# finsberg/fenicsx-beat

Measured on AMD Instinct MI355X. Metric: node_updates_per_sec, higher is better.
Workload: dtype f64

## Files before the change

### fenicsx-beat_amd/csrc/beat_ode.hip

```cpp
#include "beat_ode_kernel.h"
#include "beat_ode_jit.h"

#include <functional>


template <class Model>
static int launch_ode_run(beat_ctx* ctx, double* states, int64_t n, int64_t ld, const double* host_params,
                          int num_params, const double* ppn, int64_t pld, double t0, double dt, int64_t nsteps,
                          int nbeats, int save_freq, const int* track_idx, int ntrack, double* trace) {
  BEAT_REQUIRE(num_params == Model::NP || (host_params == nullptr && ppn == nullptr && Model::NP == 2),
               "model expects %d parameters, got %d", Model::NP, num_params);
  BEAT_REQUIRE(ntrack >= 0 && ntrack <= 8, "at most 8 tracked states");
  BEAT_REQUIRE(ntrack == 0 || (trace != nullptr && save_freq >= 1), "tracking needs a trace buffer and save_freq >= 1");
  ParamPack<Model::NP> prm;
  for (int k = 0; k < Model::NP; ++k) prm.p[k] = host_params ? host_params[k] : 1.0;
  typename Model::Derived drv = Model::derive(prm.p);
  TrackSpec tr{};
  tr.n = ntrack;
  for (int a = 0; a < ntrack; ++a) {
    BEAT_REQUIRE(track_idx[a] >= 0 && track_idx[a] < Model::NS, "tracked state %d out of range", track_idx[a]);
    tr.idx[a] = track_idx[a];
  }
  const unsigned grid = (unsigned)((n + BEAT_BLOCK - 1) / BEAT_BLOCK);
  if (ppn != nullptr) {
// ... 44 lines not shown
                                                        nsteps, nbeats, save_freq, host_track_idx, ntrack, dev_trace);
  });
  return rc == BEAT_NOT_BUILTIN ? unknown_model(model_id) : rc;
}

static unsigned ode_grid(int64_t n, int num_states) {
  unsigned grid = (unsigned)((n + BEAT_BLOCK - 1) / BEAT_BLOCK);
  static const int grid_cap_env = [] {
    const char* e = std::getenv("BEAT_ODE_GRID");
    return e ? std::atoi(e) : -1;
  }();
  static const int tile_min_states = [] {
    const char* e = std::getenv("BEAT_ODE_TILE_MIN_STATES");
    return e ? std::atoi(e) : 12;
  }();
  const int grid_cap = grid_cap_env >= 0 ? grid_cap_env : (num_states >= tile_min_states ? 0 : 24576);
  static const bool balance = [] {
    const char* e = std::getenv("BEAT_ODE_BALANCE");
    return !(e && e[0] == '0');
  }();
  if (grid_cap > 0 && grid > (unsigned)grid_cap) {
    const unsigned per_block = (grid + (unsigned)grid_cap - 1) / (unsigned)grid_cap;
    grid = (balance && per_block <= 8) ? (grid + per_block - 1) / per_block : (unsigned)grid_cap;
  }
  return grid;
}

template <class Model, bool PER_NODE, bool MARKED = false, bool SPARSE = false>
static auto launch_instance(bool have_pend, hipStream_t stream, unsigned grid, double* states, int64_t n, int64_t ld,
                            const ParamPack<Model::NP>& prm, const typename Model::Derived& drv, const double* ppn, int64_t pld, double t,
                            double dt, int v_index, double* v_copy, const PendingV& pend, const MarkedArgs& mk, const SparseRows& sp) {
  if (have_pend)
    BEAT_KERNEL((ode_step_kernel<Model, PER_NODE, true, MARKED, SPARSE>), dim3(grid), dim3(BEAT_BLOCK), 0, stream, states, n, ld, prm, drv,
                ppn, pld, t, dt, v_index, v_copy, pend, mk, sp);
  else
    BEAT_KERNEL((ode_step_kernel<Model, PER_NODE, false, MARKED, SPARSE>), dim3(grid), dim3(BEAT_BLOCK), 0, stream, states, n, ld, prm, drv,
                ppn, pld, t, dt, v_index, v_copy, pend, mk, sp);
}

template <class Model>
static int launch_ode(beat_ctx* ctx, double* states, int64_t n, int64_t ld, const double* host_params,
                      int num_params, const double* ppn, int64_t pld, double t, double dt,
                      int v_index, double* v_copy, const PendingV& pend, MarkedArgs mk = MarkedArgs{nullptr, nullptr, 0, nullptr, nullptr},
                      SparseRows sp = SparseRows{{0}, 0}) {
  BEAT_REQUIRE(num_params == Model::NP || (host_params == nullptr && ppn == nullptr && Model::NP == 2) || mk.markers != nullptr,
               "model expects %d parameters, got %d", Model::NP, num_params);
  BEAT_REQUIRE(host_params != nullptr || ppn != nullptr || mk.markers != nullptr || Model::NP == 2,
               "no parameters given: a host vector, per-node rows or parameter classes");
  if (int rc = beat_check_step_rows(Model::NS, Model::V_INDEX, v_index, v_copy, mk.markers != nullptr, pend)) return rc;
  const bool have_pend = beat_pending_has_work(pend);
  ParamPack<Model::NP> prm;
  for (int k = 0; k < Model::NP; ++k) prm.p[k] = host_params ? host_params[k] : 1.0;
  typename Model::Derived drv = Model::derive(prm.p);
  const unsigned grid = ode_grid(n, Model::NS);
  if (mk.markers != nullptr) {
    BEAT_REQUIRE(ppn == nullptr && mk.table != nullptr, "parameter classes come with a table, not with per-node rows");
    launch_instance<Model, false, true>(have_pend, ctx->stream, grid, states, n, ld, prm, drv, ppn, pld, t, dt, v_index, v_copy, pend, mk, sp);
  } else if (ppn != nullptr && sp.count > 0) {
    BEAT_REQUIRE(pld >= n, "params_ld %lld < n %lld", (long long)pld, (long long)n);
    BEAT_REQUIRE(host_params != nullptr, "sparse rows come with the uniform parameter vector");
    {
      const int rc = beat_ode_jit_launch<Model>(ctx, dim3(grid), have_pend, states, n, ld, prm, drv, ppn, pld, t, dt, v_index, v_copy, pend, mk, sp);
      if (rc != BEAT_JIT_UNAVAILABLE) return rc;
    }
    BEAT_REQUIRE(sp.count <= BEAT_MAX_SPARSE_ROWS_RT, "%d varying rows need run-time compilation, which is not available here "
                 "(beat_ode_jit_stats; at most %d rows otherwise): pass all rows (beat_ode_step)", sp.count, BEAT_MAX_SPARSE_ROWS_RT);
    launch_instance<Model, true, false, true>(have_pend, ctx->stream, grid, states, n, ld, prm, drv, ppn, pld, t, dt, v_index, v_copy, pend, mk,
                                              sp);
  } else if (ppn != nullptr) {
    BEAT_REQUIRE(pld >= n, "params_ld %lld < n %lld", (long long)pld, (long long)n);
    launch_instance<Model, true>(have_pend, ctx->stream, grid, states, n, ld, prm, drv, ppn, pld, t, dt, v_index, v_copy, pend, mk, sp);
  } else {
    launch_instance<Model, false>(have_pend, ctx->stream, grid, states, n, ld, prm, drv, ppn, pld, t, dt, v_index, v_copy, pend, mk, sp);
  }
  BEAT_LAUNCH_CHECK();
  return BEAT_OK;
}

extern "C" int beat_ode_model_info(int model_id, int* num_states, int* num_params) {
  int ns = 0, np = 0;
  const int rc = with_builtin_model(model_id, [&](auto tag) {
    using M = typename decltype(tag)::type;
    ns = M::NS;
    np = M::NP;
    return BEAT_OK;
  });
  if (rc == BEAT_NOT_BUILTIN && beat_custom_model_info(model_id, &ns, &np, nullptr) != BEAT_OK)
    return unknown_model(model_id);
  if (num_states) *num_states = ns;
  if (num_params) *num_params = np;
  return BEAT_OK;
}

static int ode_step_dispatch(beat_ctx* ctx, int model_id, double* dev_states, int64_t n, int64_t ld,
                             const double* host_params, int num_params, const double* dev_params_per_node,
                             int64_t params_ld, double t, double dt, int v_index, double* dev_v_copy,
                             const PendingV& pend, MarkedArgs mk = MarkedArgs{nullptr, nullptr, 0, nullptr, nullptr},
                             SparseRows sp = SparseRows{{0}, 0}) {
  BEAT_REQUIRE(ctx != nullptr, "null context");
  BEAT_REQUIRE(dev_states != nullptr, "null states");
  BEAT_REQUIRE(n >= 0 && ld >= n, "bad shape n=%lld ld=%lld", (long long)n, (long long)ld);
  BEAT_REQUIRE((n + BEAT_BLOCK - 1) / BEAT_BLOCK < (int64_t)0x7fffffff, "n too large");
  if (n == 0) return BEAT_OK;
  if (model_id >= BEAT_MODEL_CUSTOM_BASE) {
    BEAT_REQUIRE(sp.count == 0, "a model registered as source takes a uniform vector, all per-node rows or classes (no sparse rows)");
    int cns = 0, cnp = 0, cvi = 0;
// ... 298 lines not shown
```

### fenicsx-beat_amd/csrc/beat_ode_kernel.h

```cpp
#pragma once
#include "beat_pde_internal.h"

#include <algorithm>
#include <cmath>
#include <cstddef>
#include <cstdlib>
#include <type_traits>
#include <vector>
#include "ionic_models.h"
#include "torord_dyncl.h"


template <int NP>
struct ParamPack {
  double p[NP];
};

struct PendingV {
  const double* ring;
  int64_t fld;
  const double* alphas;
  int count;
  beat_pde_detail::GuessTerms gt;
  const double* dev_st;
// ... 39 lines not shown
};

constexpr int BEAT_MAX_SPARSE_ROWS = 16;
constexpr int BEAT_MAX_SPARSE_ROWS_RT = 4;
struct SparseRows {
  int idx[BEAT_MAX_SPARSE_ROWS];
  int count;
};

template <class Model>
struct OdeTableEntry {
  double p[Model::NP];
  typename Model::Derived d;
};

template <int... K>
struct IdxPack {
  static constexpr int count = (int)sizeof...(K);
};
template <class CT>
struct MixedParams;
template <int... K>
struct MixedParams<IdxPack<K...>> {
  const double* u;
  double v[sizeof...(K) > 0 ? sizeof...(K) : 1];
  __device__ __forceinline__ double operator[](int k) const {
    double r = u[k];
    int j = 0;
    ((r = (k == K ? v[j] : r), ++j), ...);
    return r;
  }
};
template <class D, unsigned long long DM0, unsigned long long DM1>
__device__ __forceinline__ D mix_derived(const D& du, const D& dl) {
  D d;
  constexpr int ND = (int)(sizeof(D) / sizeof(double));
  static_assert(sizeof(D) % sizeof(double) == 0 && ND <= 128, "Derived: up to 128 doubles");
  const double* a = (const double*)&du;
  const double* b = (const double*)&dl;
  double* o = (double*)&d;
#pragma unroll
  for (int j = 0; j < ND; ++j) o[j] = (((j < 64 ? DM0 : DM1) >> (j & 63)) & 1ull) ? b[j] : a[j];
  return d;
}

template <class Model, class = void>
struct beat_fm_type { using type = FastMath; };
template <class Model>
struct beat_fm_type<Model, std::void_t<typename Model::FM>> { using type = typename Model::FM; };
template <class Model, class = void>
struct beat_fm_pin_wanted : std::false_type {};
template <class Model>
struct beat_fm_pin_wanted<Model, std::void_t<decltype(Model::FM_PIN)>> : std::integral_constant<bool, Model::FM_PIN> {};
__device__ __forceinline__ double beat_any_value() {
  double x;
#ifdef __AMDGCN__
  asm volatile("" : "=v"(x));
#else
  x = 0.0;
#endif
  return x;
}
template <class Model, bool PER_NODE, bool PEND, bool MARKED = false, bool SPARSE = false, class CT = IdxPack<>,
          unsigned long long DM0 = 0, unsigned long long DM1 = 0>
__global__ __launch_bounds__(BEAT_BLOCK, (PER_NODE && CT::count == 0) ? Model::WAVES_PER_NODE : Model::WAVES) void ode_step_kernel(
    double* __restrict__ states, int64_t n, int64_t ld, ParamPack<Model::NP> prm,
    typename Model::Derived drv, const double* __restrict__ ppn, int64_t pld, double t, double dt,
    int v_index, double* __restrict__ v_copy, PendingV pend, MarkedArgs mk_arg, SparseRows sp) {
  __shared__ double etab[BEAT_EXP_TAB];
  __shared__ LogEntry ltab[128];
  static_assert(BEAT_EXP_TAB == BEAT_BLOCK, "one table entry per thread");
  etab[threadIdx.x] = beat_exp_tab_entry<beat_fm_type<Model>::type::INT_SCALE>(kExp2Tab[threadIdx.x], (int)threadIdx.x);
  if (threadIdx.x < 128) ltab[threadIdx.x] = kLogTab[threadIdx.x];
  __shared__ int cls_jn[MARKED ? BEAT_BLOCK : 1];
  __shared__ int s_pend[2];
  if (PEND && threadIdx.x == 0) {
    s_pend[0] = pend.dev_st != nullptr ? (pend.dev_st[beat_pde_detail::STOP] != 0.0 ? 1 : 0) : 1;
    s_pend[1] = pend.dev_st != nullptr ? (int)pend.dev_st[beat_pde_detail::NUPD] : -1;
  }
  __syncthreads();
  typename beat_fm_type<Model>::type fm{etab, ltab};
  if constexpr (beat_fm_pin_wanted<Model>::value) beat_fm_pin(fm);
  if (PEND && s_pend[0] == 0) return;
  const int wave_in_block = __builtin_amdgcn_readfirstlane((int)(threadIdx.x >> 6));
  for (int64_t tile = blockIdx.x;; tile += gridDim.x) {
  typedef const __attribute__((address_space(4))) char* KArgPtr;
  KArgPtr ka = (KArgPtr)__builtin_amdgcn_kernarg_segment_ptr();
  asm volatile("" : "+s"(ka));
  const PendingV& pendl = *(const PendingV*)(ka + offsetof(OdeStepKernArgHead<Model>, pend));
  const OdeStepKernArgHead<Model>& hd = *(const OdeStepKernArgHead<Model>*)ka;
  double* __restrict__ const states = hd.states;
  const int64_t n = hd.n, ld = hd.ld;
  const double* __restrict__ const ppn = hd.ppn;
  const int64_t pld = hd.pld;
  const double t = hd.t, dt = hd.dt;
  const int v_index = hd.v_index;
  double* __restrict__ const v_copy = hd.v_copy;
  (void)ppn; (void)pld; (void)v_index; (void)v_copy;
  if (tile * BEAT_BLOCK >= n) break;
  int lane_now = (int)__builtin_amdgcn_mbcnt_hi(~0u, __builtin_amdgcn_mbcnt_lo(~0u, 0u));
  asm volatile("" : "+v"(lane_now));
  const int tid = (wave_in_block << 6) + lane_now;
  const int64_t tile0 = tile * BEAT_BLOCK;
  unsigned lane_off = (unsigned)tid * 8u;
  const int64_t i = tile0 + tid;
  if (i >= n) break;
// ... 79 lines not shown
    NodeIOPending<Model::V_INDEX> io{states + tile0, ldl, lane_off, v_copy != nullptr ? v_copy + tile0 : nullptr, now.count, {}, {}, 0.0, 0.0, 0.0, 0.0, {}};
#pragma unroll
    for (int j = 0; j < BEAT_MAX_PENDING; ++j) {
      io.pp[j] = j < now.count ? __builtin_nontemporal_load(beat_at(pendl.ring + ((int64_t)j * pendl.fld + tile0), lane_off)) : beat_any_value();
      io.pa[j] = j < now.count ? pendl.alphas[j] : 0.0;
    }
    io.ge = io.gd = io.gp0 = io.gp1 = 0.0;
    if (now.gt.d != nullptr) {
      now.gt.d += tile0;
      now.gt.e += tile0;
      if (now.gt.dp[0] != nullptr) now.gt.dp[0] += tile0;
      if (now.gt.dp[1] != nullptr) now.gt.dp[1] += tile0;
      io.gt = now.gt;
      io.ge = beat_pde_detail::beat_guess_needs_e(now.gt) ? __builtin_nontemporal_load(beat_at(now.gt.e, lane_off)) : beat_any_value();
      io.gd = beat_pde_detail::beat_guess_needs_d(now.gt) ? __builtin_nontemporal_load(beat_at(now.gt.d, lane_off)) : beat_any_value();
      io.gp0 = beat_pde_detail::beat_guess_needs_dp(now.gt, 0) ? __builtin_nontemporal_load(beat_at(now.gt.dp[0], lane_off)) : beat_any_value();
      io.gp1 = beat_pde_detail::beat_guess_needs_dp(now.gt, 1) ? __builtin_nontemporal_load(beat_at(now.gt.dp[1], lane_off)) : beat_any_value();
    }
    if constexpr (PER_NODE && SPARSE && CT::count > 0) {
      MixedParams<CT> mp;
      mp.u = p_uni;
#pragma unroll
      for (int j = 0; j < CT::count; ++j) mp.v[j] = *beat_at(beat_row(ppn + tile0, j, pld), lane_off);
      if constexpr (DM0 == 0 && DM1 == 0) {
        Model::step(io, mp, d_uni, fm, t, dt);
      } else {
        const typename Model::Derived dlane = Model::derive(mp);
        const typename Model::Derived dm = mix_derived<typename Model::Derived, DM0, DM1>(d_uni, dlane);
        Model::step(io, mp, dm, fm, t, dt);
      }
    } else if (PER_NODE) {
      double pl[Model::NP];
      if (SPARSE) {
        const double* pv = p_uni;
        asm volatile("" : "+v"(pv));
#pragma unroll
        for (int k = 0; k < Model::NP; ++k) pl[k] = pv[k];
#pragma unroll
        for (int j = 0; j < BEAT_MAX_SPARSE_ROWS_RT; ++j) {
          if (j < sp.count) {
            const double vj = *beat_at(beat_row(ppn + tile0, j, pld), lane_off);
            int ij = sp.idx[j];
            asm volatile("" : "+s"(ij));
#pragma unroll
            for (int k = 0; k < Model::NP; ++k) pl[k] = k == ij ? vj : pl[k];
          }
        }
      } else {
#pragma unroll
        for (int k = 0; k < Model::NP; ++k) pl[k] = *beat_at(beat_row(ppn + tile0, k, pld), lane_off);
      }
      const typename Model::Derived dl = Model::derive(pl);
      Model::step(io, pl, dl, fm, t, dt);
    } else {
      Model::step(io, p_uni, d_uni, fm, t, dt);
    }
  } else {
    const NodeIO io{states + tile0, ldl, lane_off, nullptr, -1};
    if constexpr (PER_NODE && SPARSE && CT::count > 0) {
      MixedParams<CT> mp;
      mp.u = p_uni;
#pragma unroll
      for (int j = 0; j < CT::count; ++j) mp.v[j] = *beat_at(beat_row(ppn + tile0, j, pld), lane_off);
      if constexpr (DM0 == 0 && DM1 == 0) {
        Model::step(io, mp, d_uni, fm, t, dt);
      } else {
        const typename Model::Derived dlane = Model::derive(mp);
        const typename Model::Derived dm = mix_derived<typename Model::Derived, DM0, DM1>(d_uni, dlane);
        Model::step(io, mp, dm, fm, t, dt);
      }
    } else if (PER_NODE) {
      double pl[Model::NP];
      if (SPARSE) {
        const double* pv = p_uni;
        asm volatile("" : "+v"(pv));
#pragma unroll
        for (int k = 0; k < Model::NP; ++k) pl[k] = pv[k];
#pragma unroll
        for (int j = 0; j < BEAT_MAX_SPARSE_ROWS_RT; ++j) {
          if (j < sp.count) {
            const double vj = *beat_at(beat_row(ppn + tile0, j, pld), lane_off);
            int ij = sp.idx[j];
            asm volatile("" : "+s"(ij));
#pragma unroll
            for (int k = 0; k < Model::NP; ++k) pl[k] = k == ij ? vj : pl[k];
          }
        }
      } else {
#pragma unroll
        for (int k = 0; k < Model::NP; ++k) pl[k] = *beat_at(beat_row(ppn + tile0, k, pld), lane_off);
      }
      const typename Model::Derived dl = Model::derive(pl);
      Model::step(io, pl, dl, fm, t, dt);
    } else {
      Model::step(io, p_uni, d_uni, fm, t, dt);
    }
    if (v_copy != nullptr) v_copy[i] = states[(int64_t)v_index * ldl + i];
  }
  }
}

struct TrackSpec {
  int idx[8];
  int n;
};

template <class Model, bool PER_NODE>
__global__ __launch_bounds__(BEAT_BLOCK, 1) void ode_run_kernel(
    double* __restrict__ states, int64_t n, int64_t ld, ParamPack<Model::NP> prm, typename Model::Derived drv,
    const double* __restrict__ ppn, int64_t pld, double t0, double dt, int64_t nsteps, int nbeats, int save_freq,
    TrackSpec track, double* __restrict__ trace) {
  __shared__ double etab[BEAT_EXP_TAB];
  __shared__ LogEntry ltab[128];
  static_assert(BEAT_EXP_TAB == BEAT_BLOCK, "one table entry per thread");
  etab[threadIdx.x] = beat_exp_tab_entry<beat_fm_type<Model>::type::INT_SCALE>(kExp2Tab[threadIdx.x], (int)threadIdx.x);
  if (threadIdx.x < 128) ltab[threadIdx.x] = kLogTab[threadIdx.x];
  __syncthreads();
  typename beat_fm_type<Model>::type fm{etab, ltab};
  if constexpr (beat_fm_pin_wanted<Model>::value) beat_fm_pin(fm);
  const int64_t i = (int64_t)blockIdx.x * BEAT_BLOCK + threadIdx.x;
  if (i >= n) return;
  double y[Model::NS];
#pragma unroll
  for (int k = 0; k < Model::NS; ++k) y[k] = states[(int64_t)k * ld + i];
  double pl[PER_NODE ? Model::NP : 1];
  typename Model::Derived dl = drv;
  if (PER_NODE) {
#pragma unroll
    for (int k = 0; k < Model::NP; ++k) pl[k] = ppn[(int64_t)k * pld + i];
    dl = Model::derive((const double*)pl);
  }
  const RegIO rio{y};
  const NodeIO gio{states + (int64_t)blockIdx.x * BEAT_BLOCK, ld, threadIdx.x * 8u, nullptr, -1};
  int64_t row = 0;
  for (int beat = 0; beat < nbeats; ++beat) {
    for (int64_t j = 0; j < nsteps; ++j) {
      if (track.n > 0 && j % save_freq == 0) {
        for (int a = 0; a < track.n; ++a) {
          double v = 0.0;
#pragma unroll
          for (int k = 0; k < Model::NS; ++k)
            if (k == track.idx[a]) v = y[k];
          trace[(row * track.n + a) * n + i] = v;
        }
        ++row;
      }
// ... 23 lines not shown
```

### fenicsx-beat_amd/csrc/ionic_models.h

```cpp
#pragma once

#include <cmath>
#include <type_traits>
#include <utility>

#include "beat_common.h"


constexpr int BEAT_EXP_TAB = 256;
__device__ const double kExp2Tab[BEAT_EXP_TAB] = {
    1.0, 1.0027112750502025, 1.0054299011128027, 1.0081558981184175,
    1.0108892860517005, 1.0136300849514894, 1.016378314910953, 1.019133996077738,
    1.0218971486541166, 1.0246677928971357, 1.0274459491187637, 1.030231637686041,
    1.0330248790212284, 1.0358256936019572, 1.0386341019613787, 1.041450124688316,
    1.0442737824274138, 1.0471050958792898, 1.0499440858006872, 1.0527907730046264,
    1.0556451783605572, 1.0585073227945128, 1.061377227289262, 1.0642549128844645,
    1.0671404006768237, 1.0700337118202419, 1.0729348675259756, 1.075843889062791,
    1.0787607977571199, 1.0816856149932152, 1.0846183622133092, 1.0875590609177697,
    1.0905077326652577, 1.0934643990728858, 1.0964290818163769, 1.099401802630222,
    1.102382583307841, 1.1053714457017412, 1.1083684117236787, 1.1113735033448175,
    1.1143867425958924, 1.1174081515673693, 1.1204377524096067, 1.12347556733302,
    1.1265216186082418, 1.129575928566288, 1.1326385195987192, 1.1357094141578055,
    1.1387886347566916, 1.1418762039695616, 1.1449721444318042, 1.148076478840179,
    1.1511892299529827, 1.154310420590216, 1.1574400736337511, 1.1605782120274988,
// ... 194 lines not shown
template <bool INT_SCALE>
__device__ __forceinline__ double beat_clamp_exp_arg(double x) {
  return fmin(fmax(x, BEAT_EXP_LO), INT_SCALE ? BEAT_EXP_HI_INT : BEAT_EXP_HI);
}
__device__ __forceinline__ double beat_exp_overflow(double x, double e) { return x > BEAT_EXP_HI ? HUGE_VAL : e; }
template <bool INT_SCALE>
__device__ __forceinline__ double beat_exp_tab_entry(double t, int j) {
#ifdef __AMDGCN__
  if constexpr (INT_SCALE) return __hiloint2double(__double2hiint(t) - (j << 12), __double2loint(t));
#endif
  (void)j;
  return t;
}

__device__ __forceinline__ double beat_rcp(double x) {
  const double r = __builtin_amdgcn_rcp(x);
  const double e = fma(-x, r, 1.0);
  return fma(r, fma(e, e, e), r);
}

__device__ __forceinline__ double beat_rsqrt(double x) {
  const double r = __builtin_amdgcn_rsq(x);
  const double e = fma(-(x * r), r, 1.0);
  return fma(r * fma(e, 0.375, 0.5), e, r);
}

__device__ __forceinline__ double beat_frexp_mant(double x) {
#ifdef __AMDGCN__
  return __builtin_amdgcn_frexp_mant(x);
#else
  int e;
  return std::frexp(x, &e);
#endif
}
__device__ __forceinline__ int beat_frexp_exp(double x) {
#ifdef __AMDGCN__
  return __builtin_amdgcn_frexp_exp(x);
#else
  int e = 0;
  return std::isfinite(x) ? (std::frexp(x, &e), e) : 0;
#endif
}
__device__ __forceinline__ bool beat_pos_finite(double x) {
#ifdef __AMDGCN__
  return __builtin_amdgcn_class(x, 0x180);
#else
  return x > 0.0 && x < HUGE_VAL;
#endif
}
__device__ __forceinline__ double beat_log_special(double x) {
  const double y = x + 0.0;
  return y - __builtin_amdgcn_rsq(y);
}

__device__ __forceinline__ double beat_sconst(double c) {
#ifdef __AMDGCN__
  asm volatile("" : "+s"(c));
#endif
  return c;
}

template <bool INT_SCALE_>
struct FastMathT {
  static constexpr bool INT_SCALE = INT_SCALE_;
  const double* __restrict__ tab;
  const LogEntry* __restrict__ ltab;
  double magic = 6755399441055744.0;
  __device__ __forceinline__ double log(double x) const {
    const double xm = beat_frexp_mant(x);
    const int hi = __double2hiint(xm);
    const int e = beat_frexp_exp(x) - 1;
    const LogEntry t = ltab[(hi >> 13) & 127];
    const double m = __hiloint2double((hi & 0x000fffff) | 0x3ff00000, __double2loint(xm));
    const double r = fma(m, t.inv, -1.0);
    double p = fma(r, -1.0 / 6.0, 1.0 / 5.0);
    p = fma(r, p, -0.25);
    p = fma(r, p, 1.0 / 3.0);
    p = fma(r, p, -0.5);
    p = fma(r * r, p, r);
    const double ed = (double)e;
    const double es = __hiloint2double(beat_pos_finite(x) ? __double2hiint(ed) : __double2hiint(beat_log_special(x)), __double2loint(ed));
    return fma(es, 0.693147180559663, t.logc + fma(es, 2.8235290563031577e-13, p));
  }
  __device__ __forceinline__ double exp(double x) const {
    const double kb = fma(x, 369.3299304675746, magic);
    const double k = kb - magic;
    double r = fma(k, -0.002707606173999011, x);
    r = fma(k, -6.327543041662719e-14, r);
    const int ki = __double2loint(kb);
    const double t = tab[ki & (BEAT_EXP_TAB - 1)];
    const double r2 = r * r;
    double p = fma(r, beat_sconst(1.0 / 6.0), 0.5);
    p = fma(r2, beat_sconst(1.0 / 24.0), p);
    p = fma(r2, p, r);
#ifdef __AMDGCN__
    if constexpr (INT_SCALE) {
      const double ts = __hiloint2double(__double2hiint(t) + (int)((unsigned)ki << 12), __double2loint(t));
      return fma(ts, p, ts);
    }
#endif
    return ldexp(fma(t, p, t), ki >> 8);
  }
};

using FastMath = FastMathT<false>;
template <bool I>
__device__ __forceinline__ void beat_fm_pin(FastMathT<I>& fm) {
#ifdef __AMDGCN__
  asm volatile("" : "+v"(fm.magic));
#endif
}

__device__ __forceinline__ double beat_guard(double v) { return fabs(v) < 1.0e-4 ? copysign(1.0e-4, v) : v; }

__device__ __forceinline__ double beat_row_load(const double* p) {
#ifdef __clang__
  return __builtin_nontemporal_load(p);
#else
  return *p;
#endif
}
__device__ __forceinline__ void beat_row_store(double* p, double v) {
#ifdef __clang__
  __builtin_nontemporal_store(v, p);
#else
  *p = v;
#endif
}

template <class T>
__device__ __forceinline__ T* beat_row(T* base, int k, int64_t ld) {
#ifdef __AMDGCN__
  asm volatile("" : "+s"(ld));
#endif
  return base + (int64_t)k * ld;
// ... 4 lines not shown
#ifdef __AMDGCN__
  asm volatile("" : "+v"(byte_off));
#endif
  return (T*)((Byte*)uniform_base + byte_off);
}
struct NodeIO {
  double* __restrict__ base;
  int64_t ld;
  mutable unsigned i;
  double* __restrict__ v_copy;
  int v_index;
  __device__ __forceinline__ double load(int k) const { return beat_row_load(beat_at(beat_row(base, k, ld), i)); }
  __device__ __forceinline__ void store(int k, double v) const {
    beat_row_store(beat_at(beat_row(base, k, ld), i), v);
    if (v_copy != nullptr && k == v_index) *beat_at(v_copy, i) = v;
  }
};

constexpr int BEAT_MAX_PENDING = 6;
constexpr int BEAT_MAX_PENDING_CLASS = 12;
template <int VIDX>
struct NodeIOPending {
  double* __restrict__ base;
  int64_t ld;
  mutable unsigned i;
  double* __restrict__ v_copy;
  int npend;
  double pa[BEAT_MAX_PENDING], pp[BEAT_MAX_PENDING];
  double ge, gd, gp0, gp1;
  beat_pde_detail::GuessTerms gt;
  __device__ __forceinline__ double load(int k) const {
    double x = beat_row_load(beat_at(beat_row(base, k, ld), i));
    if (k == VIDX) {
      if (gt.d != nullptr) {
        double inc = (!gt.accumulate && gt.use_e) ? ge : 0.0;
#pragma unroll
        for (int j = 0; j < BEAT_MAX_PENDING; ++j)
          if (j < npend) inc = fma(pa[j], pp[j], inc);
        beat_pde_detail::beat_guess_record(gt, beat_at(gt.d, i), beat_at(gt.e, i), inc, gd, gp0, gp1, ge);
        return x + inc;
      }
#pragma unroll
      for (int j = 0; j < BEAT_MAX_PENDING; ++j)
        if (j < npend) x = fma(pa[j], pp[j], x);
    }
    return x;
  }
  __device__ __forceinline__ void store(int k, double v) const {
    beat_row_store(beat_at(beat_row(base, k, ld), i), v);
    if (k == VIDX && v_copy != nullptr) *beat_at(v_copy, i) = v;
  }
};

struct RegIO {
  double* y;
  __device__ __forceinline__ double load(int k) const { return y[k]; }
  __device__ __forceinline__ void store(int k, double v) const { y[k] = v; }
};

struct SimpleOde {
  static constexpr int NS = 2, NP = 2, V_INDEX = 0;
  static constexpr bool REGISTER_LOOP = true;
  static constexpr int WAVES = BEAT_ODE_WAVES;
  static constexpr int WAVES_PER_NODE = BEAT_ODE_WAVES_PER_NODE;
  struct Derived {};
  __host__ __device__ static Derived derive(const double*) { return {}; }
  template <class IO>
  __device__ static __forceinline__ void step(const IO& io, const double* p, const Derived&, const FastMath&,
                                              double, double dt) {
    const double v = io.load(0), s = io.load(1);
    io.store(0, v - p[0] * s * dt);
    io.store(1, s + p[1] * v * dt);
  }
};

struct FhnDemo {
  static constexpr int NS = 2, NP = 10, V_INDEX = 1;
  static constexpr bool REGISTER_LOOP = true;
  static constexpr int WAVES = BEAT_ODE_WAVES;
  static constexpr int WAVES_PER_NODE = BEAT_ODE_WAVES_PER_NODE;
  struct Derived {};
  __host__ __device__ static Derived derive(const double*) { return {}; }
  template <class IO>
  __device__ static __forceinline__ void step(const IO& io, const double* p, const Derived&, const FastMath&,
                                              double t, double dt) {
    const double s = io.load(0), V = io.load(1);
    const double V_peak = p[0], V_rest = p[1], a = p[2], b = p[3], c_1 = p[4], c_2 = p[5],
                 c_3 = p[6], stim_amplitude = p[7], stim_duration = p[8], stim_start = p[9];
    const double V_amp = V_peak - V_rest;
    const double i_Stim = (t >= stim_start && t <= stim_start + stim_duration) ? stim_amplitude : 0.0;
    const double ds_dt = b * (-c_3 * s + (V - V_rest));
    const double V_th = V_amp * a + V_rest;
    const double I = -s * (c_2 / V_amp) * (V - V_rest) +
                     (((c_1 / (V_amp * V_amp)) * (V - V_rest)) * (V - V_th)) * (-V + V_peak);
    const double dV_dt = I + i_Stim;
    io.store(0, s + dt * ds_dt);
    io.store(1, V + dt * dV_dt);
  }
};

struct FhnReadme {
  static constexpr int NS = 2, NP = 11, V_INDEX = 1;
  static constexpr bool REGISTER_LOOP = true;
  static constexpr int WAVES = BEAT_ODE_WAVES;
  static constexpr int WAVES_PER_NODE = BEAT_ODE_WAVES_PER_NODE;
  struct Derived {};
  __host__ __device__ static Derived derive(const double*) { return {}; }
  template <class IO>
  __device__ static __forceinline__ void step(const IO& io, const double* p, const Derived&, const FastMath&,
                                              double t, double dt) {
    const double s = io.load(0), v = io.load(1);
    const double c_1 = p[0], c_2 = p[1], c_3 = p[2], a = p[3], b = p[4], v_amp = p[5],
                 v_rest = p[6], v_peak = p[7], stim_amplitude = p[8], stim_duration = p[9],
                 stim_start = p[10];
    const double i_app = (t > stim_start && t < stim_start + stim_duration) ? stim_amplitude : 0.0;
    const double ds_dt = b * (-c_3 * s + (v - v_rest));
    const double v_th = v_amp * a + v_rest;
    const double I = -s * (c_2 / v_amp) * (v - v_rest) +
                     (((c_1 / (v_amp * v_amp)) * (v - v_rest)) * (v - v_th)) * (-v + v_peak);
    const double dV_dt = I + i_app;
    io.store(0, ds_dt * dt + s);
    io.store(1, v + dV_dt * dt);
  }
};

#ifdef __clang__
#pragma clang fp contract(fast)
#endif
struct Tp06Grl1 {
  static constexpr int NS = 19, NP = 53, V_INDEX = 17;
  static constexpr bool ACCESSOR_PARAMS = true;
  static constexpr bool REGISTER_LOOP = true;
#ifndef BEAT_TP06_WAVES
#define BEAT_TP06_WAVES 4
#endif
  static constexpr int WAVES = BEAT_TP06_WAVES;
  static constexpr int WAVES_PER_NODE = BEAT_ODE_WAVES_PER_NODE;
  using FM = FastMath;
  static constexpr bool FM_PIN = true;
  enum S { Xr1, Xr2, Xs, m, h, j, d, f, f2, fCass, s, r, R_prime, Ca_i, Ca_SR, Ca_ss, Na_i, V, K_i };
  enum P {
    P_kna, g_K1, g_Kr, g_Ks, g_Na, g_bna, g_CaL, g_bca, g_to, P_NaK, K_mk, K_mNa, K_NaCa, K_sat,
    alpha, gamma, Km_Ca, Km_Nai, g_pCa, K_pCa, g_pK, Ca_o, k1_prime, k2_prime, k3, k4, EC, max_sr,
    min_sr, V_rel, V_xfer, K_up, V_leak, Vmax_up, Buf_c, K_buf_c, Buf_sr, K_buf_sr, Buf_ss,
    K_buf_ss, V_sr, V_ss, Na_o, R, T, F, Cm, V_c, stim_start, stim_period, stim_duration,
    stim_amplitude, K_o
  };

  struct Derived {
    double RTF, FRT, halfRTF, sqrtKo, gK1s, gKrs, KoPk, cCaL, NaK_B, Nao3, A2c, kNaCaQ, gm1,
        cVF, c1, c2, c3, c4, c5, Kup2, BKc, BKsr, BKss, dsr;
  };
  template <class P>
  __host__ __device__ static Derived derive(const P& p) {
    Derived q;
    q.RTF = p[R] * p[T] / p[F];
    q.FRT = p[F] / (p[R] * p[T]);
    q.halfRTF = 0.5 * p[R] * p[T] / p[F];
    q.sqrtKo = sqrt(p[K_o] / 5.4);
    q.gK1s = p[g_K1] * q.sqrtKo;
    q.gKrs = p[g_Kr] * q.sqrtKo;
    q.KoPk = p[K_o] + p[P_kna] * p[Na_o];
    q.cCaL = p[g_CaL] * 4.0 * (p[F] * p[F]) / (p[R] * p[T]);
    q.NaK_B = p[P_NaK] * p[K_o] / (p[K_o] + p[K_mk]);
    q.Nao3 = p[Na_o] * p[Na_o] * p[Na_o];
    q.A2c = q.Nao3 * p[alpha];
    q.kNaCaQ = p[K_NaCa] / ((p[Km_Nai] * p[Km_Nai] * p[Km_Nai] + q.Nao3) * (p[Km_Ca] + p[Ca_o]));
    q.gm1 = p[gamma] - 1.0;
    q.cVF = p[Cm] / (p[V_c] * p[F]);
    q.c1 = p[Cm] / (2.0 * p[V_c] * p[F]);
    q.c2 = p[V_sr] / p[V_c];
    q.c3 = p[Cm] / (2.0 * p[V_ss] * p[F]);
    q.c4 = p[V_sr] / p[V_ss];
    q.c5 = p[V_c] / p[V_ss];
    q.Kup2 = p[K_up] * p[K_up];
    q.BKc = p[Buf_c] * p[K_buf_c];
    q.BKsr = p[Buf_sr] * p[K_buf_sr];
    q.BKss = p[Buf_ss] * p[K_buf_ss];
    q.dsr = p[max_sr] - p[min_sr];
    return q;
  }

  __device__ static __forceinline__ double rcp(double x) { return beat_rcp(x); }
  __device__ static __forceinline__ void rcp2(double a, double b, double& ia, double& ib) {
    const double r = rcp(a * b);
    ia = r * b;
    ib = r * a;
  }
  __device__ static __forceinline__ void rcp3(double a, double b, double c, double& ia, double& ib, double& ic) {
    const double ab = a * b;
    const double r = rcp(ab * c);
    ic = r * ab;
    const double t = r * c;
    ia = t * b;
    ib = t * a;
  }
  __device__ static __forceinline__ void rcp4(double a, double b, double c, double d, double& ia, double& ib,
                                              double& ic, double& id) {
    const double ab = a * b, cd = c * d;
    const double r = rcp(ab * cd);
    const double rab = r * cd, rcd = r * ab;
    ia = rab * b;
    ib = rab * a;
    ic = rcd * d;
    id = rcd * c;
  }
  __device__ static __forceinline__ double grl1(const FM& fm, double y, double fy, double J, double dt) {
    return y + ((fabs(J) > 1e-8) ? fy * (beat_exp_overflow(J * dt, fm.exp(beat_clamp_exp_arg<FM::INT_SCALE>(J * dt))) - 1.0) * rcp(J) : fy * dt);
  }
  __device__ static __forceinline__ double phi_small(double z) {
    double ph = fma(z, beat_sconst(1.0 / 362880.0), beat_sconst(1.0 / 40320.0));
    ph = fma(z, ph, beat_sconst(1.0 / 5040.0));
    ph = fma(z, ph, beat_sconst(1.0 / 720.0));
    ph = fma(z, ph, beat_sconst(1.0 / 120.0));
    ph = fma(z, ph, beat_sconst(1.0 / 24.0));
    ph = fma(z, ph, beat_sconst(1.0 / 6.0));
    ph = fma(z, ph, 0.5);
    return fma(z, ph, 1.0);
  }
  __device__ static __forceinline__ double advance(const FM& fm, double y, double fy, double J, double dt) {
    const double z = J * dt;
    if (fabs(z) <= 0.0625) return fma(fy * dt, phi_small(z), y);
    return grl1(fm, y, fy, J, dt);
  }
  __device__ static __forceinline__ double phi7(double z) {
    double ph = fma(z, beat_sconst(1.0 / 40320.0), beat_sconst(1.0 / 5040.0));
    ph = fma(z, ph, beat_sconst(1.0 / 720.0));
    ph = fma(z, ph, beat_sconst(1.0 / 120.0));
    ph = fma(z, ph, beat_sconst(1.0 / 24.0));
    ph = fma(z, ph, beat_sconst(1.0 / 6.0));
    ph = fma(z, ph, 0.5);
    return fma(z, ph, 1.0);
  }
  __device__ static __forceinline__ double gate(const FM& fm, double y, double inf, double rtau, double dt) {
    return y + (inf - y) * (1.0 - fm.exp(fmax(-dt * rtau, BEAT_EXP_LO)));
  }

#define BEAT_FENCE() __builtin_amdgcn_sched_barrier(0)

  template <class IO, class P>
  __device__ static __forceinline__ void step(const IO& io, const P& p, const Derived& q, const FM& fm,
                                              double t, double dt) {
    const double v = io.load(V);
    constexpr double EXP_M3 = 0.049787068367863944;
    constexpr double EXP_2P5 = 12.182493960703473;
    constexpr double EXP_M4P5 = 0.011108996538242306;
    constexpr double EXP_1P3 = 3.6692966676192444;
    constexpr double EXP_3 = 20.085536923187668;
    constexpr double EXP_M3P2 = 0.04076220397836621;
    constexpr double EXP_M12 = 6.14421235332821e-06;
    constexpr double EXP_7 = 1096.6331584284585;
    constexpr double EXP_1 = 2.718281828459045;
    constexpr double EXP_4 = 54.598150033144236;
    constexpr double EXP_M4 = 0.01831563888873418;
    constexpr double EXP_M26_7 = 0.0243728440732796;
    constexpr double EXP_20_7 = 17.41170806332765;
    constexpr double EXP_5 = 148.4131591025766;
    constexpr double EXP_5_6 = 2.300975890892825;
    constexpr double EXP_20_6 = 28.03162489452614;
    constexpr double EXP_M1 = 0.36787944117144233;
    constexpr double EXP_P02 = 1.0202013400267558;

    const double oXr1 = io.load(Xr1), oXr2 = io.load(Xr2), oXs = io.load(Xs), om = io.load(m), oh = io.load(h),
                 oj = io.load(j), od = io.load(d), of = io.load(f), of2 = io.load(f2), ofCass = io.load(fCass),
                 os = io.load(s), orr = io.load(r);
    const double gNa = p[g_Na] * (om * om * om) * oh * oj;
    const double gKr = q.gKrs * oXr1 * oXr2;
    const double gKs = p[g_Ks] * (oXs * oXs);
    const double gto = p[g_to] * orr * os;
    const double gates_CaL = q.cCaL * od * of * of2 * ofCass;
    const double vCai = io.load(Ca_i), vCaSR = io.load(Ca_SR), vCass = io.load(Ca_ss), vNai = io.load(Na_i),
                 vKi = io.load(K_i), vR = io.load(R_prime);

    const double E20 = fm.exp(0.05 * v), E7 = fm.exp(v * (1.0 / 7.0));
    double I20, I7;
    rcp2(E20, E7, I20, I7);
    const double E10 = E20 * E20, I10 = I20 * I20;
    const double E5 = E10 * E10, I5 = I10 * I10;
    const double I6 = fm.exp(v * (-1.0 / 6.0));
    BEAT_FENCE();

    {
      double inf1, inf2;
      rcp2(1.0 + EXP_M26_7 * I7, 1.0 + fm.exp((v + 88.0) * (1.0 / 24.0)), inf1, inf2);
      const double rtau1 = (1.0 + EXP_M4P5 * I10) * (1.0 + fm.exp((v + 30.0) * (1.0 / 11.5))) * (1.0 / 2700.0);
      io.store(Xr1, gate(fm, oXr1, inf1, rtau1, dt));
      const double rtau2 = (1.0 + EXP_M3 * I20) * (1.0 + EXP_M3 * E20) * (1.0 / 3.36);
      io.store(Xr2, gate(fm, oXr2, inf2, rtau2, dt));
    }
    BEAT_FENCE();
    {
      const double D = sqrt(1.0 + EXP_5_6 * I6) * (1.0 + fm.exp((v - 35.0) * (1.0 / 15.0)));
      double inf, rnum;
      rcp2(1.0 + fm.exp((-5.0 - v) * (1.0 / 14.0)), 1400.0 + 80.0 * D, inf, rnum);
      io.store(Xs, gate(fm, oXs, inf, D * rnum, dt));
// ... 25 lines not shown
        ah_bh = 0.77 * rbh;
        aj_bj = 0.6 * fm.exp(0.057 * v) * rbj;
      }
      const double h_inf = rh * rh;
      io.store(h, gate(fm, oh, h_inf, ah_bh, dt));
      io.store(j, gate(fm, oj, h_inf, aj_bj, dt));
    }
    BEAT_FENCE();
    {
      const double da = 1.0 + fm.exp((-35.0 - v) * (1.0 / 13.0));
      const double db = 1.0 + EXP_1 * E5;
      const double dc = 1.0 + EXP_2P5 * I20;
      const double num = (1.4 + 0.25 * da) * 1.4 * dc + da * db;
      double inf, rnum;
      rcp2(1.0 + fm.exp((-8.0 - v) * (1.0 / 7.5)), num, inf, rnum);
      io.store(d, gate(fm, od, inf, da * db * dc * rnum, dt));
    }
    BEAT_FENCE();
    {
      const double v27sq = (v + 27.0) * (v + 27.0);
      const double db = 1.0 + EXP_3 * E10;
      const double da1 = 1.0 + EXP_1P3 * I10;
      const double dab1 = da1 * db;
      const double num1 = (1102.5 * fm.exp(v27sq * (-1.0 / 225.0)) + 20.0) * dab1 + 200.0 * db + 180.0 * da1;
      const double da2 = 1.0 + EXP_2P5 * I10;
      const double dab2 = da2 * db;
      const double num2 = 562.0 * fm.exp(v27sq * (-1.0 / 240.0)) * dab2 + 31.0 * db + 80.0 * da2;
      double inf1, rnum1, rinf2, rnum2;
      rcp4(1.0 + EXP_20_7 * E7, num1, 1.0 + EXP_5 * E7, num2, inf1, rnum1, rinf2, rnum2);
      io.store(f, gate(fm, of, inf1, dab1 * rnum1, dt));
      io.store(f2, gate(fm, of2, 0.67 * rinf2 + 0.33, dab2 * rnum2, dt));
    }
    BEAT_FENCE();
    {
      const double ds_ = 1.0 + EXP_M4 * E5;
      const double num = (85.0 * fm.exp((v + 45.0) * (v + 45.0) * (-1.0 / 320.0)) + 3.0) * ds_ + 5.0;
      double s_inf, rnum, r_inf, rtau_r;
      rcp4(1.0 + EXP_4 * E5, num, 1.0 + EXP_20_6 * I6,
           9.5 * fm.exp((v + 40.0) * (v + 40.0) * (-1.0 / 1800.0)) + 0.8, s_inf, rnum, r_inf, rtau_r);
      io.store(s, gate(fm, os, s_inf, ds_ * rnum, dt));
      io.store(r, gate(fm, orr, r_inf, rtau_r, dt));
    }
    BEAT_FENCE();

    {
      const double c2 = 1.0 + (vCass * 20.0) * (vCass * 20.0);
      double rc2, rt;
      rcp2(c2, 80.0 + 2.0 * c2, rc2, rt);
      io.store(fCass, gate(fm, ofCass, 0.6 * rc2 + 0.4, c2 * rt, dt));
    }

    double rNai, rKi, rCai, rKs;
    rcp4(vNai, vKi, vCai, vKi + p[P_kna] * vNai, rNai, rKi, rCai, rKs);
    const double E_Na = q.RTF * fm.log(p[Na_o] * rNai);
    const double E_K = q.RTF * fm.log(p[K_o] * rKi);
    const double E_Ks = q.RTF * fm.log(q.KoPk * rKs);
    const double E_Ca = q.halfRTF * fm.log(p[Ca_o] * rCai);
    const double u = v - E_K;
    BEAT_FENCE();

    double I_tot, I_K, dI_dV, sum_du;
    {
      const double G = fm.exp(0.02 * u);
      const double G2 = G * G, G4 = G2 * G2, G5 = G4 * G, G10 = G5 * G5, G25 = G10 * G10 * G5;
      const double e1 = EXP_M12 * (G2 * G);
      const double e2 = EXP_P02 * fm.exp(0.0002 * u);
      const double e3 = EXP_M1 * G5;
      double e4, r1, rG1;
      rcp3(G25, 1.0 + e1, G25 + 1.0, e4, r1, rG1);
      const double aK1 = 0.1 * r1;
      const double daK1 = -0.06 * aK1 * e1 * r1;
      const double rD = G25 * rG1;
      const double bK1 = (3.0 * e2 + e3) * rD;
      const double dbK1 = (0.0006 * e2 + 0.1 * e3 + 0.5 * e4 * bK1) * rD;
      const double epK = fm.exp((25.0 - v) * (1.0 / 5.98));
      double rab, rpK;
      rcp2(aK1 + bK1, 1.0 + epK, rab, rpK);
      const double xK1 = aK1 * rab;
      const double dxK1 = (daK1 * bK1 - aK1 * dbK1) * rab * rab;
      const double i_K1 = q.gK1s * xK1 * u;
      const double i_p_K = p[g_pK] * u * rpK;
      I_K = i_K1 + gto * u + gKr * u + i_p_K;
      sum_du = q.gK1s * (dxK1 * u + xK1) + gto + gKr + p[g_pK] * rpK;
      dI_dV = sum_du + p[g_pK] * u * epK * (1.0 / 5.98) * rpK * rpK + gKs;
      I_K += gKs * (v - E_Ks);
      I_tot = I_K;
    }
    BEAT_FENCE();

    const double vF = v * q.FRT;
    const double e5 = fm.exp(-0.1 * vF);
    const double e5_2 = e5 * e5, e5_4 = e5_2 * e5_2, e5_8 = e5_4 * e5_4;
    const double e6 = e5_8 * e5_2;
    const double eg = fm.exp(p[gamma] * vF);
    const double eg1 = eg * e6;
    double rNaK, rNaKm, rS;
    rcp3(1.0 + 0.1245 * e5 + 0.0353 * e6, vNai + p[K_mNa], 1.0 + p[K_sat] * eg1, rNaK, rNaKm, rS);
    const double i_NaK = q.NaK_B * vNai * rNaKm * rNaK;
    const double di_NaK_dNai = q.NaK_B * p[K_mNa] * rNaKm * rNaKm * rNaK;
    dI_dV += i_NaK * q.FRT * (0.01245 * e5 + 0.0353 * e6) * rNaK;
    const double A1 = (vNai * vNai * vNai) * p[Ca_o], A2 = q.A2c * vCai;
    const double NNaCa = eg * A1 - eg1 * A2;
    const double kS = q.kNaCaQ * rS;
    const double i_NaCa = kS * NNaCa;
    dI_dV += kS * q.FRT * ((p[gamma] * eg * A1 - q.gm1 * eg1 * A2) - NNaCa * p[K_sat] * q.gm1 * eg1 * rS);
    const double di_NaCa_dNai = kS * eg * 3.0 * (vNai * vNai) * p[Ca_o];
    const double di_NaCa_dCai = -kS * eg1 * q.A2c;
    const double i_Na_tot = (gNa + p[g_bna]) * (v - E_Na);
    dI_dV += gNa + p[g_bna] + p[g_bca];
    const double i_b_Ca = p[g_bca] * (v - E_Ca);
    I_tot += i_NaK + i_NaCa + i_Na_tot + i_b_Ca;
    BEAT_FENCE();

    const double w15 = v - 15.0;
    const double xCaL = 2.0 * w15 * q.FRT;
    const double eCaL = fm.exp(xCaL);
    const bool nearCaL = fabs(xCaL) < 1.0e-2;
    double rDc, rpCa;
    rcp2(nearCaL ? 1.0 : eCaL - 1.0, vCai + p[K_pCa], rDc, rpCa);
    const double NCaL = 0.25 * vCass * eCaL - p[Ca_o];
    double i_CaL = gates_CaL * w15 * NCaL * rDc;
    double dCaL_dV = gates_CaL * (NCaL * rDc + w15 * (2.0 * q.FRT) * eCaL * (p[Ca_o] - 0.25 * vCass) * rDc * rDc);
    double di_CaL_dCass = gates_CaL * w15 * 0.25 * eCaL * rDc;
    if (nearCaL) {
      const double x2 = xCaL * xCaL;
      const double phi = 1.0 + xCaL * (-0.5 + xCaL * (1.0 / 12.0 + x2 * (-1.0 / 720.0 + x2 * (1.0 / 30240.0))));
      const double dphi = -0.5 + xCaL * (1.0 / 6.0 + x2 * (-1.0 / 180.0 + x2 * (1.0 / 5040.0)));
      const double B = phi * q.halfRTF;
      i_CaL = gates_CaL * NCaL * B;
      dCaL_dV = gates_CaL * (0.25 * vCass * eCaL * phi + NCaL * dphi);
      di_CaL_dCass = gates_CaL * 0.25 * eCaL * B;
    }
    dI_dV += dCaL_dV;
    const double i_p_Ca = p[g_pCa] * vCai * rpCa;
    const double di_pCa_dCai = p[g_pCa] * p[K_pCa] * rpCa * rpCa;
    I_tot += i_CaL + i_p_Ca;
    BEAT_FENCE();

    const double tmod = t - floor(t / p[stim_period]) * p[stim_period];
    const double i_Stim =
        (tmod >= p[stim_start] && tmod <= p[stim_start] + p[stim_duration]) ? p[stim_amplitude] : 0.0;
    {
      const double J_V = -dI_dV;
      const double J_Ki = -(sum_du * q.RTF * rKi + gKs * q.RTF * rKs) * q.cVF;
      const double J_Nai = -((gNa + p[g_bna]) * q.RTF * rNai + 3.0 * di_NaK_dNai + 3.0 * di_NaCa_dNai) * q.cVF;
      io.store(V, advance(fm, v, -(I_tot + i_Stim), J_V, dt));
      io.store(K_i, advance(fm, vKi, -(I_K + i_Stim - 2.0 * i_NaK) * q.cVF, J_Ki, dt));
      io.store(Na_i, advance(fm, vNai, -(i_Na_tot + 3.0 * i_NaK + 3.0 * i_NaCa) * q.cVF, J_Nai, dt));
    }
    BEAT_FENCE();

    const double qup = q.Kup2 * rCai * rCai;
    double rup, rbc, rCaSR, rbsr, rbss;
    rcp3(1.0 + qup, vCai + p[K_buf_c], vCaSR, rup, rbc, rCaSR);
    rcp2(vCaSR + p[K_buf_sr], vCass + p[K_buf_ss], rbsr, rbss);
    const double zsr = (p[EC] * rCaSR) * (p[EC] * rCaSR);
    const double gci = q.BKc * rbc * rbc, gsr = q.BKsr * rbsr * rbsr, gss = q.BKss * rbss * rbss;
    double rz, Fr_i, Fr_sr, Fr_ss;
    rcp4(1.0 + zsr, 1.0 + gci, 1.0 + gsr, 1.0 + gss, rz, Fr_i, Fr_sr, Fr_ss);
    const double i_up = p[Vmax_up] * rup;
    const double di_up_dCai = i_up * 2.0 * qup * rCai * rup;
    const double i_leak = p[V_leak] * (vCaSR - vCai);
    const double i_xfer = p[V_xfer] * (vCass - vCai);
    {
      const double T_i = -(i_b_Ca + i_p_Ca - 2.0 * i_NaCa) * q.c1 + (i_leak - i_up) * q.c2 + i_xfer;
      const double dT_i = -(p[g_bca] * q.halfRTF * rCai + di_pCa_dCai - 2.0 * di_NaCa_dCai) * q.c1 +
                          (-p[V_leak] - di_up_dCai) * q.c2 - p[V_xfer];
      io.store(Ca_i, advance(fm, vCai, T_i * Fr_i, dT_i * Fr_i + T_i * (Fr_i * Fr_i * 2.0 * gci * rbc), dt));
    }
    BEAT_FENCE();
    const double kcasr = p[max_sr] - q.dsr * rz;
    const double dkcasr = -2.0 * q.dsr * zsr * rCaSR * rz * rz;
    const double rkc = rcp(kcasr);
    const double k1 = p[k1_prime] * rkc;
    const double dk1 = -k1 * dkcasr * rkc;
    const double k2 = p[k2_prime] * kcasr;
    const double css2 = vCass * vCass;
    const double rO = rcp(p[k3] + k1 * css2);
    const double O = k1 * css2 * vR * rO;
    const double dO_dk1 = css2 * vR * p[k3] * rO * rO;
    const double dO_dCass = 2.0 * vCass * k1 * vR * p[k3] * rO * rO;
    const double dsrss = vCaSR - vCass;
    const double i_rel = p[V_rel] * O * dsrss;
    io.store(R_prime, advance(fm, vR, -k2 * vCass * vR + p[k4] * (1.0 - vR), -vCass * k2 - p[k4], dt));
    {
      const double T_sr = i_up - (i_rel + i_leak);
      const double dT_sr = -(p[V_rel] * (dO_dk1 * dk1 * dsrss + O) + p[V_leak]);
      io.store(Ca_SR, advance(fm, vCaSR, T_sr * Fr_sr, dT_sr * Fr_sr + T_sr * (Fr_sr * Fr_sr * 2.0 * gsr * rbsr), dt));
    }
    BEAT_FENCE();
    {
      const double T_ss = -i_CaL * q.c3 + i_rel * q.c4 - i_xfer * q.c5;
      const double dT_ss = -di_CaL_dCass * q.c3 + p[V_rel] * (dO_dCass * dsrss - O) * q.c4 - p[V_xfer] * q.c5;
      io.store(Ca_ss, advance(fm, vCass, T_ss * Fr_ss, dT_ss * Fr_ss + T_ss * (Fr_ss * Fr_ss * 2.0 * gss * rbss), dt));
// ... 8 lines not shown
```

Before: 11.38 billion.

## Hoist uniform stimulus to host and batch log with wave-uniform fast path

```diff
diff --git a/fenicsx-beat_amd/csrc/beat_ode.hip b/fenicsx-beat_amd/csrc/beat_ode.hip
--- a/fenicsx-beat_amd/csrc/beat_ode.hip
+++ b/fenicsx-beat_amd/csrc/beat_ode.hip
@@ -120,6 +120,7 @@
   ParamPack<Model::NP> prm;
   for (int k = 0; k < Model::NP; ++k) prm.p[k] = host_params ? host_params[k] : 1.0;
   typename Model::Derived drv = Model::derive(prm.p);
+  if constexpr (beat_host_stim<Model>::value) drv.i_stim = Model::stim_host(prm.p, t);
   const unsigned grid = ode_grid(n, Model::NS);
   if (mk.markers != nullptr) {
     BEAT_REQUIRE(ppn == nullptr && mk.table != nullptr, "parameter classes come with a table, not with per-node rows");
diff --git a/fenicsx-beat_amd/csrc/beat_ode_kernel.h b/fenicsx-beat_amd/csrc/beat_ode_kernel.h
--- a/fenicsx-beat_amd/csrc/beat_ode_kernel.h
+++ b/fenicsx-beat_amd/csrc/beat_ode_kernel.h
@@ -115,6 +115,10 @@
 struct beat_fm_pin_wanted : std::false_type {};
 template <class Model>
 struct beat_fm_pin_wanted<Model, std::void_t<decltype(Model::FM_PIN)>> : std::integral_constant<bool, Model::FM_PIN> {};
+template <class Model, class = void>
+struct beat_host_stim : std::false_type {};
+template <class Model>
+struct beat_host_stim<Model, std::void_t<decltype(Model::HOST_STIM)>> : std::integral_constant<bool, Model::HOST_STIM> {};
 __device__ __forceinline__ double beat_any_value() {
   double x;
 #ifdef __AMDGCN__
@@ -300,6 +304,8 @@
       }
       const typename Model::Derived dl = Model::derive(pl);
       Model::step(io, pl, dl, fm, t, dt);
+    } else if constexpr (beat_host_stim<Model>::value) {
+      Model::step(io, p_uni, d_uni, fm, BeatLaunchStim{}, dt);
     } else {
       Model::step(io, p_uni, d_uni, fm, t, dt);
     }
@@ -340,6 +346,8 @@
       }
       const typename Model::Derived dl = Model::derive(pl);
       Model::step(io, pl, dl, fm, t, dt);
+    } else if constexpr (beat_host_stim<Model>::value) {
+      Model::step(io, p_uni, d_uni, fm, BeatLaunchStim{}, dt);
     } else {
       Model::step(io, p_uni, d_uni, fm, t, dt);
     }
diff --git a/fenicsx-beat_amd/csrc/ionic_models.h b/fenicsx-beat_amd/csrc/ionic_models.h
--- a/fenicsx-beat_amd/csrc/ionic_models.h
+++ b/fenicsx-beat_amd/csrc/ionic_models.h
@@ -270,6 +270,20 @@
   const double y = x + 0.0;
   return y - __builtin_amdgcn_rsq(y);
 }
+__device__ __forceinline__ bool beat_pos_normal(double x) {
+#ifdef __AMDGCN__
+  return __builtin_amdgcn_class(x, 0x100);
+#else
+  return x >= 2.2250738585072014e-308 && x < HUGE_VAL;
+#endif
+}
+__device__ __forceinline__ bool beat_wave_all(bool c) {
+#ifdef __AMDGCN__
+  return __builtin_amdgcn_ballot_w64(!c) == 0;
+#else
+  return c;
+#endif
+}
 
 __device__ __forceinline__ double beat_sconst(double c) {
 #ifdef __AMDGCN__
@@ -284,21 +298,44 @@
   const double* __restrict__ tab;
   const LogEntry* __restrict__ ltab;
   double magic = 6755399441055744.0;
-  __device__ __forceinline__ double log(double x) const {
-    const double xm = beat_frexp_mant(x);
-    const int hi = __double2hiint(xm);
-    const int e = beat_frexp_exp(x) - 1;
+  __device__ __forceinline__ double log_core(int hi, int lo, double es) const {
     const LogEntry t = ltab[(hi >> 13) & 127];
-    const double m = __hiloint2double((hi & 0x000fffff) | 0x3ff00000, __double2loint(xm));
+    const double m = __hiloint2double((hi & 0x000fffff) | 0x3ff00000, lo);
     const double r = fma(m, t.inv, -1.0);
     double p = fma(r, -1.0 / 6.0, 1.0 / 5.0);
     p = fma(r, p, -0.25);
     p = fma(r, p, 1.0 / 3.0);
     p = fma(r, p, -0.5);
     p = fma(r * r, p, r);
-    const double ed = (double)e;
-    const double es = __hiloint2double(beat_pos_finite(x) ? __double2hiint(ed) : __double2hiint(beat_log_special(x)), __double2loint(ed));
     return fma(es, 0.693147180559663, t.logc + fma(es, 2.8235290563031577e-13, p));
+  }
+  template <int N>
+  __device__ __forceinline__ void logn(const double (&x)[N], double (&out)[N]) const {
+    bool normal = true;
+#pragma unroll
+    for (int j = 0; j < N; ++j) normal = normal && beat_pos_normal(x[j]);
+    if (beat_wave_all(normal)) {
+#pragma unroll
+      for (int j = 0; j < N; ++j) {
+        const int hi = __double2hiint(x[j]);
+        out[j] = log_core(hi, __double2loint(x[j]), (double)((hi >> 20) - 1023));
+      }
+      return;
+    }
+#pragma unroll
+    for (int j = 0; j < N; ++j) {
+      const double xm = beat_frexp_mant(x[j]);
+      const int e = beat_frexp_exp(x[j]) - 1;
+      const double ed = (double)e;
+      const double es = __hiloint2double(beat_pos_finite(x[j]) ? __double2hiint(ed) : __double2hiint(beat_log_special(x[j])), __double2loint(ed));
+      out[j] = log_core(__double2hiint(xm), __double2loint(xm), es);
+    }
+  }
+  __device__ __forceinline__ double log(double x) const {
+    const double a[1] = {x};
+    double o[1];
+    logn(a, o);
+    return o[0];
   }
   __device__ __forceinline__ double exp(double x) const {
     const double kb = fma(x, 369.3299304675746, magic);
@@ -409,6 +446,8 @@
   }
 };
 
+struct BeatLaunchStim {};
+
 struct RegIO {
   double* y;
   __device__ __forceinline__ double load(int k) const { return y[k]; }
@@ -507,6 +546,7 @@
   struct Derived {
     double RTF, FRT, halfRTF, sqrtKo, gK1s, gKrs, KoPk, cCaL, NaK_B, Nao3, A2c, kNaCaQ, gm1,
         cVF, c1, c2, c3, c4, c5, Kup2, BKc, BKsr, BKss, dsr;
+    double i_stim;
   };
   template <class P>
   __host__ __device__ static Derived derive(const P& p) {
@@ -535,7 +575,20 @@
     q.BKsr = p[Buf_sr] * p[K_buf_sr];
     q.BKss = p[Buf_ss] * p[K_buf_ss];
     q.dsr = p[max_sr] - p[min_sr];
+    q.i_stim = 0.0;
     return q;
+  }
+  static constexpr bool HOST_STIM = true;
+  template <class P>
+  __device__ static __forceinline__ double stim(const P& p, const Derived&, double t) {
+    const double tmod = t - floor(t / p[stim_period]) * p[stim_period];
+    return (tmod >= p[stim_start] && tmod <= p[stim_start] + p[stim_duration]) ? p[stim_amplitude] : 0.0;
+  }
+  template <class P>
+  __device__ static __forceinline__ double stim(const P&, const Derived& q, BeatLaunchStim) { return q.i_stim; }
+  __host__ static double stim_host(const double* p, double t) {
+    const double tmod = std::fma(-p[stim_period], std::floor(t / p[stim_period]), t);
+    return (tmod >= p[stim_start] && tmod <= p[stim_start] + p[stim_duration]) ? p[stim_amplitude] : 0.0;
   }
 
   __device__ static __forceinline__ double rcp(double x) { return beat_rcp(x); }
@@ -595,9 +648,9 @@
 
 #define BEAT_FENCE() __builtin_amdgcn_sched_barrier(0)
 
-  template <class IO, class P>
+  template <class IO, class P, class T>
   __device__ static __forceinline__ void step(const IO& io, const P& p, const Derived& q, const FM& fm,
-                                              double t, double dt) {
+                                              const T& t, double dt) {
     const double v = io.load(V);
     constexpr double EXP_M3 = 0.049787068367863944;
     constexpr double EXP_2P5 = 12.182493960703473;
@@ -729,10 +782,13 @@
 
     double rNai, rKi, rCai, rKs;
     rcp4(vNai, vKi, vCai, vKi + p[P_kna] * vNai, rNai, rKi, rCai, rKs);
-    const double E_Na = q.RTF * fm.log(p[Na_o] * rNai);
-    const double E_K = q.RTF * fm.log(p[K_o] * rKi);
-    const double E_Ks = q.RTF * fm.log(q.KoPk * rKs);
-    const double E_Ca = q.halfRTF * fm.log(p[Ca_o] * rCai);
+    const double lx[4] = {p[Na_o] * rNai, p[K_o] * rKi, q.KoPk * rKs, p[Ca_o] * rCai};
+    double lg[4];
+    fm.logn(lx, lg);
+    const double E_Na = q.RTF * lg[0];
+    const double E_K = q.RTF * lg[1];
+    const double E_Ks = q.RTF * lg[2];
+    const double E_Ca = q.halfRTF * lg[3];
     const double u = v - E_K;
     BEAT_FENCE();
 
@@ -814,9 +870,7 @@
     I_tot += i_CaL + i_p_Ca;
     BEAT_FENCE();
 
-    const double tmod = t - floor(t / p[stim_period]) * p[stim_period];
-    const double i_Stim =
-        (tmod >= p[stim_start] && tmod <= p[stim_start] + p[stim_duration]) ? p[stim_amplitude] : 0.0;
+    const double i_Stim = stim(p, q, t);
     {
       const double J_V = -dI_dV;
       const double J_Ki = -(sum_du * q.RTF * rKi + gKs * q.RTF * rKs) * q.cVF;
```

After: 11.51 billion (median of 6 runs). +1.1%, better.
